# rohithr87/CILRS-Autonomous-Driving-CARLA

Measured on AMD Instinct MI355X. Metric: frames/sec CILRS train batch=128, higher is better.
Workload: dtype f32; 1 GPU; CILRS ResNet-34 train step (fwd+loss+bwd+Adam), Config A, 200x88 RGB, B=128/GPU, fp32; global_batch=128, parallelism=single

## Files before the change

### cilrs-autonomous-driving-carla_amd/cilrs_mi355/_lib.py

```python
from __future__ import annotations

import ctypes as C
import os

_HERE = os.path.dirname(os.path.abspath(__file__))
LIB_PATH = os.environ.get("CILRS_LIB") or os.path.join(_HERE, "libcilrs_hip.so")

c_float_p = C.POINTER(C.c_float)
vp = C.c_void_p
sz = C.c_size_t
i32 = C.c_int
i64 = C.c_int64
f32 = C.c_float
f64 = C.c_double
u64 = C.c_uint64


class Buffers(C.Structure):
    _fields_ = [("params", vp), ("grads", vp), ("bn_running", vp), ("bn_nbt", vp),
                ("workspace", vp)]


class AdamArgs(C.Structure):
    _fields_ = [("exp_avg", vp), ("exp_avg_sq", vp), ("lr", C.c_double), ("beta1", C.c_double),
# ... 157 lines not shown
    "cilrs_batch_assemble": (i32, [vp, i64, vp, vp, vp, vp, vp, i32, i32, i32, vp, vp, vp, vp, vp,
                                   vp]),
    "cilrs_augment_weather_u8": (i32, [vp, vp, vp, i32, i32, i32, vp, vp, vp]),
    "cilrs_batch_assemble_weather": (i32, [vp, i64, vp, vp, vp, vp, vp, vp, i32, i32, i32, vp, vp, vp,
                                           vp, vp, vp]),
    "cilrs_augment_view_u8": (i32, [vp, vp, vp, vp, i32, i32, i32, vp, vp, vp]),
    "cilrs_batch_assemble_view": (i32, [vp, i64, vp, vp, vp, vp, vp, vp, vp, i32, i32, i32, vp, vp,
                                        vp, vp, vp, vp]),
    "cilrs_replay_state_doubles": (i32, []),
    "cilrs_replay_metric_doubles": (i32, []),
    "cilrs_replay_begin": (i32, [C.POINTER(ReplayConfig), i32, i32, i64, vp, vp, vp, vp, vp, vp, vp,
                                 vp, vp]),
    "cilrs_replay_step": (i32, [C.POINTER(ReplayConfig), i32, i32, vp, vp, vp, i64, vp, vp, vp, vp,
                                vp, vp, vp, vp]),
    "cilrs_replay_finish": (i32, [C.POINTER(ReplayConfig), i32, i32, vp, vp, vp, i64, vp, vp, vp, vp,
                                  vp, vp]),
    "cilrs_eval_acc_doubles": (i32, []),
    "cilrs_eval_accumulate": (i32, [vp, vp, vp, vp, vp, i32, vp, vp, vp]),
    "cilrs_net_profile_enable": (i32, [vp, i32]),
    "cilrs_net_profile_collect": (i32, [vp]),
    "cilrs_net_profile_count": (i32, [vp]),
    "cilrs_net_profile_entry": (i32, [vp, i32, C.c_char_p, i32, C.POINTER(C.c_longlong),
                                      C.POINTER(f64), C.POINTER(f64), C.POINTER(f64)]),
    "cilrs_net_profile_reset": (i32, [vp]),
    "cilrs_conv2d_fwd": (i32, [vp, vp, vp] + [i32] * 11 + [vp, sz, vp]),
    "cilrs_conv2d_dgrad": (i32, [vp, vp, vp, vp] + [i32] * 11 + [vp, sz, vp]),
    "cilrs_conv2d_fwd_stats": (i32, [vp, vp, vp, vp, C.POINTER(i32)] + [i32] * 10 + [vp, sz, vp]),
    "cilrs_conv2d_dgrad_bnbwd": (i32, [vp] * 7 + [i32, vp, C.POINTER(i32)] + [i32] * 10
                                 + [vp, sz, vp]),
    "cilrs_conv2d_takes_classes": (i32, [i32] * 9 + [sz, i32]),
    "cilrs_conv2d_plan_info": (i32, [i32] * 9 + [sz, i32, i32] + [C.POINTER(i32)] * 4),
    "cilrs_net_conv_classes": (i32, [vp, i32, C.POINTER(i32), C.POINTER(i32)]),
    "cilrs_conv2d_wgrad_scratch_floats": (sz, [i32] * 9),
    "cilrs_conv2d_wgrad": (i32, [vp, vp, vp, vp] + [i32] * 10 + [vp]),
    "cilrs_conv2d_16_scratch_halfs": (sz, [i32] * 8),
    "cilrs_conv2d_fwd_16": (i32, [vp, vp, vp, vp] + [i32] * 9 + [vp, vp]),
    "cilrs_conv2d_dgrad_16": (i32, [vp, vp, vp, vp] + [i32] * 9 + [vp, vp]),
    "cilrs_conv2d_wgrad_16_scratch_floats": (sz, [i32] * 8),
    "cilrs_conv2d_wgrad_16": (i32, [vp, vp, vp, vp] + [i32] * 9 + [vp, vp]),
    "cilrs_conv2d_train_16": (i32, [vp] * 9 + [i32, vp] + [i32] * 12 + [vp, vp]),
    "cilrs_conv2d_infer_16": (i32, [vp] * 5 + [i32] * 11 + [vp]),
    "cilrs_stem_fold_16": (i32, [vp, vp, vp, vp, i32, vp]),
    "cilrs_stem_infer_16": (i32, [vp, vp, vp, vp, i32, i32, i32, i32, vp]),
    "cilrs_maxpool_infer_16": (i32, [vp, vp, i32, i32, i32, i32, i32, vp]),
    "cilrs_avgpool_infer_16": (i32, [vp, vp, i32, i32, i32, i32, i32, vp]),
    "cilrs_bn16_train_fwd": (i32, [vp, i32, i32, vp, vp, vp, vp, vp, C.c_float, C.c_float, vp, i32,
                                   vp, vp, vp, i32, vp]),
    "cilrs_bn16_bwd": (i32, [vp, vp, vp, i32, i32, vp, vp, i32, vp, vp, vp, vp, vp, vp, i32, vp]),
    "cilrs_conv2d_wino_split": (i32, [vp, vp, vp, vp, vp, i32, i32, i32, i32, i32, vp, sz, vp, vp, vp]),
    "cilrs_conv2d_wino_scratch_floats": (sz, [i32, i32]),
    "cilrs_conv2d_wino_fwd": (i32, [vp, vp, vp, i32, i32, i32, i32, i32, vp, vp]),
    "cilrs_conv2d_wino_fold_fwd": (i32, [vp, vp, vp, vp, vp, vp, i32, i32, i32, i32, i32, i32, i32,
                                         vp, vp]),
    "cilrs_wino_filter_transform": (i32, [vp, vp, i32, i32, i32, vp]),
    "cilrs_conv2d_wino_stamps": (i32, [vp]),
    "cilrs_conv2d_wino_pre": (i32, [vp, vp, vp, vp, i32, i32, i32, i32, i32, vp]),
    "cilrs_conv2d_wino_dgrad": (i32, [vp, vp, vp, vp, i32, i32, i32, i32, i32, vp, vp]),
    "cilrs_conv2d_wino_wgrad_scratch_floats": (sz, [i32, i32, i32, i32, i32]),
    "cilrs_conv2d_wino_wgrad": (i32, [vp, vp, vp, i32, i32, i32, i32, i32, vp, sz, vp]),
    "cilrs_bn_partial_floats": (sz, [i32]),
    "cilrs_variant_bn_stats_doubles": (sz, [i32]),
    "cilrs_variant_bn_stats_info": (i32, [i32, i32, C.POINTER(i32), C.POINTER(sz), C.POINTER(sz)]),
    "cilrs_net_bn_layer_info": (i32, [vp, i32, C.POINTER(sz), C.POINTER(i32), C.POINTER(i32),
                                      C.POINTER(i32)]),
    "cilrs_net_forward_bn_stats": (i32, [vp, C.POINTER(Buffers), vp, C.c_long, C.c_long, C.c_long, C.c_long, vp, vp]),
    "cilrs_bn_stats_finalize": (i32, [i32, vp, i32, vp, vp, vp]),
# ... 62 lines not shown
```

### cilrs-autonomous-driving-carla_amd/csrc/common.h

```cpp
#pragma once
#include <hip/hip_runtime.h>
#include <stdint.h>
#include <stddef.h>
#include "../../include/cilrs_hip.h"

namespace cilrs {

typedef float f32x4 __attribute__((ext_vector_type(4)));
typedef float f32x16 __attribute__((ext_vector_type(16)));

void set_error(const char* fmt, ...);
const char* last_error();

#define CILRS_CHECK(cond, ...)                   \
    do {                                         \
        if (!(cond)) {                           \
            ::cilrs::set_error(__VA_ARGS__);     \
            return 1;                            \
        }                                        \
    } while (0)

#define CILRS_HIP(expr)                                                                 \
    do {                                                                                \
        hipError_t e_ = (expr);                                                         \
// ... 99 lines not shown
#if defined(__HIPCC__)
__device__ __forceinline__ void wave_priority(const int mode) {
    if (mode == 0) return;
    int p;
    if (mode == 1) p = (int)(blockIdx.x >> 8) & 3;
    else p = (int)__builtin_amdgcn_s_getreg((3 << 11) | 4) & 3;
    p = __builtin_amdgcn_readfirstlane(p);
    if (p == 0) __builtin_amdgcn_s_setprio(0);
    else if (p == 1) __builtin_amdgcn_s_setprio(1);
    else if (p == 2) __builtin_amdgcn_s_setprio(2);
    else __builtin_amdgcn_s_setprio(3);
}
__device__ __forceinline__ void wave_stagger(const int mode) {
    if (mode < 16) return;
    const int units = mode - 16;
    const int k = (int)((blockIdx.x >> 8) % 5u);
    for (int i = 0; i < k * units; ++i) __builtin_amdgcn_s_sleep(1);
}
#endif
int wave_priority_mode();

struct WgradArgs {
    const float* x;
    const float* dy;
    float* dw;
    float* slabs;
    int N, H, W, Cin;
    int Ho, Wo, Cout;
    int KH, KW, stride, pad;
    int x_ld, dy_ld;
    int Cin_dst;
    int accumulate;
    int prio_mode;
};
size_t wgrad_scratch_floats(const WgradArgs& a);
int launch_conv_wgrad(const WgradArgs& a, hipStream_t s);

size_t bn_partial_floats(int C);
int launch_bn_train_fwd(const float* y, int M, int C, const float* gamma, const float* beta,
                        float* running_mean, float* running_var, long long* nbt, float momentum,
                        float eps, const float* residual, int relu, float* stats, float* partial,
                        float* z, int pre_nblk, hipStream_t s, void* z16 = nullptr,
                        double* acc_head = nullptr, double* acc = nullptr);
constexpr int kBnStatsHead = 2, kBnStatsRows = 4;
int launch_bn_train_stats(const float* y, int M, int C, double* acc, float* partial, hipStream_t s);
constexpr int kMaxConvs = 56;
struct BnEvalTable {
    int n;
    int C[kMaxConvs];
    unsigned gamma[kMaxConvs], beta[kMaxConvs];
    unsigned rm[kMaxConvs], rv[kMaxConvs];
    unsigned stats[kMaxConvs];
};
int launch_bn_eval_stats_all(const BnEvalTable& t, const float* params, const float* bn_running,
                             float* ws, float eps, hipStream_t s);
struct BnStatsTable {
    int n;
    int C[kMaxConvs];
    unsigned rm[kMaxConvs], rv[kMaxConvs];
    unsigned head[kMaxConvs], sums[kMaxConvs];
};
int launch_bn_stats_finalize(const BnStatsTable& t, const double* table, int estimator,
                             float* bn_running, long long* bn_nbt, hipStream_t s);
int launch_bn_eval_fwd(const float* y, int M, int C, const float* gamma, const float* beta,
                       const float* running_mean, const float* running_var, float eps,
                       const float* residual, int relu, float* stats, float* z, hipStream_t s);
int launch_bn_bwd(const float* dz, const float* z, const float* y, int M, int C,
                  const float* gamma, const float* stats, int relu, float* dgamma, float* dbeta,
                  int accumulate, float* coef, float* partial, float* dy, float* g_out,
// ... 567 lines not shown
```

### cilrs-autonomous-driving-carla_amd/csrc/conv_wgrad.hip

```cpp
#include "common.h"

#include <stdlib.h>

namespace cilrs {

namespace {

constexpr int BKP = 32;

template <int BT, bool TAP_UNIFORM, bool PIN>
__global__ __launch_bounds__(256, 2) void conv_wgrad_kernel(const WgradArgs a, const int Mpix,
                                                            const int splits, const int tiles_ci,
                                                            const int Ncols, const int ntiles_x,
                                                            const int ntiles_co,
                                                            const int xcd_group) {
    constexpr int WT = BT / 2, T = WT / 32;
    constexpr int QPR = BT / 4;
    constexpr int RPP = 256 / QPR;
    constexpr int PASSES = BKP / RPP;
    constexpr int PITCH = BT + 4;

    extern __shared__ __attribute__((aligned(16))) float smem[];
    float* As = smem;
    float* Bs = smem + 2 * BKP * PITCH;

    const int tid = threadIdx.x, lane = tid & 63, wave = tid >> 6;
    const int l31 = lane & 31, lh = lane >> 5;
    const int wm = wave >> 1, wn = wave & 1;
    wave_priority(a.prio_mode < 16 ? a.prio_mode : 0);

    int logical = (int)blockIdx.x;
    if (xcd_group) {
        const int nwg = (int)gridDim.x, bid = (int)blockIdx.x;
        const int q = nwg >> 3, r = nwg & 7, xcd = bid & 7;
        const int base = xcd < r ? xcd * (q + 1) : r * (q + 1) + (xcd - r) * q;
        logical = base + (bid >> 3);
    }
    const int ntile = logical % ntiles_x;
    const int co0 = ((logical / ntiles_x) % ntiles_co) * BT;
    const int z = logical / (ntiles_x * ntiles_co);

    const int KT = (Mpix + BKP - 1) / BKP;
    const int per = (KT + splits - 1) / splits;
    const int kt_begin = z * per;
    const int kt_end = min(KT, kt_begin + per);
    const int nt = max(kt_end - kt_begin, 0);

    const int q = tid % QPR, rr = tid / QPR;

    int tap, ci, col0;
    bool col_ok;
    if constexpr (TAP_UNIFORM) {
        tap = ntile / tiles_ci;
        ci = (ntile - tap * tiles_ci) * BT + q * 4;
        col0 = tap * a.Cin + (ntile - tap * tiles_ci) * BT;
        col_ok = true;
    } else {
        col0 = ntile * BT;
        const int j = col0 + q * 4;
        tap = j / a.Cin;
        ci = j - tap * a.Cin;
        col_ok = j < Ncols;
    }
    const int kh = tap / a.KW, kw = tap - kh * a.KW;
    const int HoWo = a.Ho * a.Wo;

    const int dn = BKP / HoWo, drem = BKP - dn * HoWo;
    const int doh = drem / a.Wo, dow = drem - doh * a.Wo;
    int cn[PASSES], coh[PASSES], cow[PASSES], cp[PASSES];
#pragma unroll
    for (int i = 0; i < PASSES; ++i) {
        const int p = kt_begin * BKP + rr + RPP * i;
        cp[i] = p;
        cn[i] = p / HoWo;
        const int rem = p - cn[i] * HoWo;
        coh[i] = rem / a.Wo;
        cow[i] = rem - coh[i] * a.Wo;
    }
    const __amdgpu_buffer_rsrc_t rsDy = __builtin_amdgcn_make_buffer_rsrc(
        (void*)a.dy, 0, (int)(unsigned)((size_t)Mpix * a.dy_ld * sizeof(float)), 0x00020000);
    const __amdgpu_buffer_rsrc_t rsX = __builtin_amdgcn_make_buffer_rsrc(
        (void*)a.x, 0, (int)(unsigned)((size_t)a.N * a.H * a.W * a.x_ld * sizeof(float)),
        0x00020000);
    const unsigned dyq = (unsigned)(co0 + q * 4) * 4u;
    const unsigned dy_pitch = (unsigned)a.dy_ld * 4u;

    auto load_tile = [&](f32x4(&ra)[PASSES], f32x4(&rb)[PASSES]) {
#pragma unroll
        for (int i = 0; i < PASSES; ++i) {
            const int h = coh[i] * a.stride - a.pad + kh, w = cow[i] * a.stride - a.pad + kw;
            const bool ok = col_ok && cp[i] < Mpix && h >= 0 && w >= 0 && h < a.H && w < a.W;
            const unsigned xo =
                ok ? (unsigned)(((cn[i] * a.H + h) * a.W + w) * a.x_ld + ci) * 4u : 0xFFFFFFFFu;
            ra[i] = __builtin_bit_cast(
                f32x4, __builtin_amdgcn_raw_buffer_load_b128(
                           rsDy, (int)((unsigned)cp[i] * dy_pitch + dyq), 0, 0));
            rb[i] = __builtin_bit_cast(
                f32x4, __builtin_amdgcn_raw_buffer_load_b128(rsX, (int)xo, 0, 0));
            cp[i] += BKP;
            cow[i] += dow;
            int c1 = cow[i] >= a.Wo;
            cow[i] -= c1 ? a.Wo : 0;
            coh[i] += doh + c1;
            int c2 = coh[i] >= a.Ho;
            coh[i] -= c2 ? a.Ho : 0;
            cn[i] += dn + c2;
        }
    };
    auto store_tile = [&](int buf, const f32x4(&ra)[PASSES], const f32x4(&rb)[PASSES]) {
#pragma unroll
        for (int i = 0; i < PASSES; ++i) {
            const int row = rr + RPP * i;
            *reinterpret_cast<f32x4*>(As + (buf * BKP + row) * PITCH + q * 4) = ra[i];
            *reinterpret_cast<f32x4*>(Bs + (buf * BKP + row) * PITCH + q * 4) = rb[i];
        }
    };

    f32x16 acc[T][T];
#pragma unroll
    for (int i = 0; i < T; ++i)
#pragma unroll
        for (int j = 0; j < T; ++j)
#pragma unroll
            for (int r = 0; r < 16; ++r) acc[i][j][r] = 0.f;

    auto compute = [&](int buf) {
        if constexpr (T == 2) {
            const float* Ab = As + buf * BKP * PITCH + lh * PITCH + wm * WT + 2 * l31;
            const float* Bb = Bs + buf * BKP * PITCH + lh * PITCH + wn * WT + 2 * l31;
#pragma unroll
            for (int s = 0; s < BKP / 2; ++s) {
                const float2 av = *reinterpret_cast<const float2*>(Ab + 2 * s * PITCH);
                const float2 bv = *reinterpret_cast<const float2*>(Bb + 2 * s * PITCH);
                acc[0][0] = __builtin_amdgcn_mfma_f32_32x32x2f32(av.x, bv.x, acc[0][0], 0, 0, 0);
                acc[0][1] = __builtin_amdgcn_mfma_f32_32x32x2f32(av.x, bv.y, acc[0][1], 0, 0, 0);
                acc[1][0] = __builtin_amdgcn_mfma_f32_32x32x2f32(av.y, bv.x, acc[1][0], 0, 0, 0);
                acc[1][1] = __builtin_amdgcn_mfma_f32_32x32x2f32(av.y, bv.y, acc[1][1], 0, 0, 0);
            }
// ... 129 lines not shown
        __shared__ float red1[256];
        const int opb = 256 / G;
        const int g = threadIdx.x / opb, ol = threadIdx.x - g * opb;
        const size_t idx = (size_t)blockIdx.x * opb + ol;
        float v = 0.f;
        if (idx < n_src) {
            const float* base = slabs + idx;
            float acc[4] = {0.f, 0.f, 0.f, 0.f};
            int sidx = g;
            for (; sidx + 3 * G < splits; sidx += 4 * G) {
#pragma unroll
                for (int u = 0; u < 4; ++u) acc[u] += base[(size_t)(sidx + u * G) * n_src];
            }
            for (; sidx < splits; sidx += G) acc[0] += base[(size_t)sidx * n_src];
            v = (acc[0] + acc[1]) + (acc[2] + acc[3]);
        }
        if (G > 1) {
            red1[threadIdx.x] = v;
            __syncthreads();
            if (g == 0) {
                for (int k = 1; k < G; ++k) v += red1[k * opb + ol];
            }
        }
        if (g == 0 && idx < n_src) {
            const int ci = (int)(idx % cin);
            if (ci < cin_dst) {
                const size_t o = (idx / cin) * cin_dst + ci;
                dw[o] = accumulate ? dw[o] + v : v;
            }
        }
    }
}

struct WPlan { int bt; bool uniform; int tiles_ci; int ntiles; int ncols; int splits; };

double wplan_cost(double flops, int tiles, int splits, int bt, size_t out_floats) {
    static const float r128[2] = {105.f, 120.f};
    static const float r64[4] = {60.f, 85.f, 96.f, 103.f};
    const int occ = bt == 128 ? 2 : 4;
    const float* rate = bt == 128 ? r128 : r64;
    const long blocks = (long)tiles * splits;
    const long per_cu = (blocks + 255) / 256;
    const double unit = flops / (double)blocks;
    const long full = per_cu / occ, rem = per_cu % occ;
    double t = 0.0;
    if (full) t += full * unit * 256.0 * occ / (rate[occ - 1] * 1e6);
    if (rem) t += unit * 256.0 * rem / (rate[rem - 1] * 1e6);
    t += (full + (rem ? 1 : 0)) * 3.0;
    t += 4.0 + (double)out_floats * 4.0 * (2.0 * splits + 1.0) / 3.5e6;
    return t;
}

WPlan plan(const WgradArgs& a) {
    WPlan best;
    const int taps = a.KH * a.KW;
    const int Mpix = a.N * a.Ho * a.Wo;
    const int KT = cdiv(Mpix, BKP);
    const bool uniform = (a.Cin % 64) == 0;
    const size_t out_floats = (size_t)a.Cout * taps * a.Cin;
    const double flops = 2.0 * Mpix * (double)out_floats;
    static const int env_bt = experiment_env("CILRS_WGRAD_BT", 0);
    static const int env_target = experiment_env("CILRS_WGRAD_TARGET", 0);
    double bc = 1e30;
    for (int bt = 64; bt <= 128; bt += 64) {
        if (bt == 128 && !(uniform && a.Cin % 128 == 0 && a.Cout % 128 == 0)) continue;
        if (env_bt && bt != env_bt) continue;
        WPlan p;
        p.bt = bt; p.uniform = uniform; p.ncols = taps * a.Cin;
        if (uniform) { p.tiles_ci = a.Cin / bt; p.ntiles = taps * p.tiles_ci; }
        else { p.tiles_ci = 1; p.ntiles = cdiv(p.ncols, bt); }
        const int tiles = p.ntiles * (a.Cout / bt);
        const int max_splits = KT / 4 > 0 ? KT / 4 : 1;
        for (int budget = 256; budget <= 2048; budget += 256) {
            if (env_target && budget != ((env_target + 255) / 256) * 256) continue;
            int splits = budget / tiles;
            if (splits < 1) splits = 1;
            if (splits > max_splits) splits = max_splits;
            const int per = cdiv(KT, splits);
            splits = cdiv(KT, per);
            const double c = wplan_cost(flops, tiles, splits, bt, out_floats);
            if (c < bc) { bc = c; best = p; best.splits = splits; }
        }
    }
    return best;
}

}

size_t wgrad_scratch_floats(const WgradArgs& a) {
    const WPlan p = plan(a);
    return (size_t)p.splits * a.Cout * p.ncols;
}

int launch_conv_wgrad(const WgradArgs& a_in, hipStream_t s) {
    WgradArgs a = a_in;
    a.prio_mode = wave_priority_mode();
    CILRS_CHECK(a.Cout % 64 == 0, "conv_wgrad: Cout=%d must be a multiple of 64", a.Cout);
    CILRS_CHECK(a.Cin % 4 == 0 && a.x_ld % 4 == 0 && a.dy_ld % 4 == 0,
                "conv_wgrad: Cin/x_ld/dy_ld must be multiples of 4");
    CILRS_CHECK(a.slabs != nullptr, "conv_wgrad: scratch slabs missing");
    CILRS_CHECK((size_t)a.N * a.H * a.W * a.x_ld * sizeof(float) < (1ull << 32) &&
                    (size_t)a.N * a.Ho * a.Wo * a.dy_ld * sizeof(float) < (1ull << 32),
                "conv_wgrad: tensor larger than 4 GB");
    CILRS_CHECK(((uintptr_t)a.x & 15) == 0 && ((uintptr_t)a.dy & 15) == 0 &&
                    ((uintptr_t)a.slabs & 15) == 0,
                "conv_wgrad: pointers must be 16-byte aligned");
    const WPlan p = plan(a);
    const int Mpix = a.N * a.Ho * a.Wo;
    const int ntiles_co = a.Cout / p.bt;
    static const int xcd = experiment_env("CILRS_WGRAD_XCD", 1);
    dim3 grid(p.ntiles * ntiles_co * p.splits, 1, 1);
    const size_t lds = (size_t)4 * BKP * (p.bt + 4) * sizeof(float);
    static const bool pin = experiment_env("CILRS_WGRAD_PIN", 1) != 0;
    if (p.bt == 128) {
        if (set_max_dynamic_lds(reinterpret_cast<const void*>(&conv_wgrad_kernel<128, true, true>), (int)lds) ||
            set_max_dynamic_lds(reinterpret_cast<const void*>(&conv_wgrad_kernel<128, true, false>), (int)lds))
            return 1;
        if (pin)
            conv_wgrad_kernel<128, true, true><<<grid, 256, lds, s>>>(a, Mpix, p.splits,
                                                                      p.tiles_ci, p.ncols, p.ntiles, ntiles_co, xcd);
        else
            conv_wgrad_kernel<128, true, false><<<grid, 256, lds, s>>>(a, Mpix, p.splits,
                                                                       p.tiles_ci, p.ncols, p.ntiles, ntiles_co, xcd);
    } else if (p.uniform) {
        if (pin)
            conv_wgrad_kernel<64, true, true><<<grid, 256, lds, s>>>(a, Mpix, p.splits,
                                                                     p.tiles_ci, p.ncols, p.ntiles, ntiles_co, xcd);
        else
            conv_wgrad_kernel<64, true, false><<<grid, 256, lds, s>>>(a, Mpix, p.splits,
                                                                      p.tiles_ci, p.ncols, p.ntiles, ntiles_co, xcd);
    } else {
        conv_wgrad_kernel<64, false, false><<<grid, 256, lds, s>>>(a, Mpix, p.splits, p.tiles_ci,
                                                                   p.ncols, p.ntiles, ntiles_co, xcd);
    }
    CILRS_LAUNCH_CHECK();
    const size_t n_src = (size_t)a.Cout * p.ncols;
    if (a.Cin == a.Cin_dst && n_src % 4 == 0 && ((uintptr_t)a.dw & 15) == 0) {
        const size_t nvec = n_src / 4;
        int G = 1;
        while (G < 16 && nvec * G < 131072 && 8 * G <= p.splits) G *= 2;
        const int opb = 256 / G;
        wgrad_reduce_kernel<4><<<(int)((nvec + opb - 1) / opb), 256, 0, s>>>(
            a.slabs, a.dw, p.splits, n_src, a.Cin, a.Cin_dst, a.accumulate, G);
    } else {
        int G = 1;
        while (G < 16 && n_src * G < 262144 && 8 * G <= p.splits) G *= 2;
        const int opb = 256 / G;
        wgrad_reduce_kernel<1><<<(int)((n_src + opb - 1) / opb), 256, 0, s>>>(
            a.slabs, a.dw, p.splits, n_src, a.Cin, a.Cin_dst, a.accumulate, G);
    }
    CILRS_LAUNCH_CHECK();
    return 0;
}

int launch_wgrad_reduce(const float* slabs, float* dw, int splits, size_t n, int accumulate,
                        hipStream_t s) {
    CILRS_CHECK(n % 4 == 0 && ((uintptr_t)dw & 15) == 0 && ((uintptr_t)slabs & 15) == 0,
                "wgrad_reduce: n %% 4, 16-byte aligned buffers");
    const size_t nvec = n / 4;
    int G = 1;
    while (G < 16 && nvec * G < 131072 && 8 * G <= splits) G *= 2;
    const int opb = 256 / G;
    wgrad_reduce_kernel<4><<<(int)((nvec + opb - 1) / opb), 256, 0, s>>>(slabs, dw, splits, n, 0, 0,
                                                                        accumulate, G);
    CILRS_LAUNCH_CHECK();
    return 0;
// ... 4 lines not shown
```

### cilrs-autonomous-driving-carla_amd/csrc/net.hip

```cpp
#include "common.h"
#include "../../include/cilrs_hip.h"

#include <math.h>
#include <stdarg.h>
#include <stdio.h>
#include <stdlib.h>
#include <string.h>

#include <algorithm>
#include <map>
#include <memory>
#include <mutex>
#include <set>
#include <string>
#include <vector>

namespace cilrs {

static thread_local char g_err[1024] = "";
void set_error(const char* fmt, ...) {
    va_list ap;
    va_start(ap, fmt);
    vsnprintf(g_err, sizeof(g_err), fmt, ap);
    va_end(ap);
// ... 530 lines not shown
        WinoArgs wa = wino_args(net, g, c.cout, c.cin);
        wa.x = dy; wa.U = ws + net->wino_base + net->wino_table.ud[e]; wa.y = dx; wa.addend = addend;
        wa.no_tail = (overlap_configured(net) && !experiment_env("CILRS_WINO_DGRAD_TAIL", 0)) ? 1 : 0;
        wa.slabs = ws + net->ksplit; wa.slab_floats = net->ksplit_floats;
        wa.scratch_partial = ws + net->bn_partial;
        if (bwd_nblk) *bwd_nblk = 0;
        if (bn_of && bwd_nblk) {
            wa.bwd_z = ws + bn_of->z; wa.bwd_y = ws + bn_of->y; wa.bwd_stats = ws + bn_of->stats;
            wa.bwd_relu = bn_relu; wa.bwd_partial = ws + net->bn_partial;
            *bwd_nblk = wino_rows(net->B, g.H, g.W, c.cin, wa.no_tail, c.cout, net->ksplit_floats);
        }
        RUN(net, label(), conv_flops(c, g), conv_bytes(net, c, g, 4, 4, 4, true), s,
            launch_conv_wino(wa, s));
        return 0;
    }
    DgradArgs a = dgrad_args(net->B, g.H, g.W, c.cin, c.cout, c.k, c.stride, c.pad);
    a.dy = dy; a.w = w; a.dx = dx; a.addend = addend;
    if (bn_of && bwd_nblk) {
        a.bwd_z = ws + bn_of->z; a.bwd_y = ws + bn_of->y; a.bwd_stats = ws + bn_of->stats;
        a.bwd_relu = bn_relu; a.bwd_partial = ws + net->bn_partial; a.bwd_nblk = bwd_nblk;
        *bwd_nblk = 0;
    }
    a.scratch = ws + net->ksplit; a.scratch_floats = net->ksplit_floats;
    a.force_cfg = -1;
    RUN(net, label(), conv_flops(c, g), conv_bytes(net, c, g, 4, 4, 4), s, launch_conv_dgrad(a, s));
    return 0;
}

static bool wino_wgrad_on(const ConvT& c) {
    static const int env = env_int("CILRS_WINO_WGRAD", 1);
    return env != 0 && wino_wgrad_supported(c.cin, c.cout, c.k, c.stride, c.pad);
}

int conv_wgrad(cilrs_net* net, const ConvT& c, const ConvG& g, const float* x, int x_cin,
               const float* dy, float* dw, float* ws, hipStream_t s) {
    auto label = [&] { return std::string("conv_wgrad.") + kGroupName[c.group]; };
    if (x_cin == c.cin && !net->bf16_train && wino_wgrad_on(c)) {
        WinoWgradArgs wa;
        memset(&wa, 0, sizeof(wa));
        wa.x = x; wa.dy = dy; wa.dw = dw; wa.slabs = ws + net->slabs;
        wa.N = net->B; wa.H = g.H; wa.W = g.W; wa.C = c.cin; wa.K = c.cout;
        CILRS_CHECK(wino_wgrad_scratch_floats(net->B, g.H, g.W, c.cin, c.cout) <= net->slabs_floats,
                    "Winograd wgrad scratch too small");
        RUN(net, label(), conv_flops(c, g), conv_bytes(net, c, g, 4, 4, 4), s,
            launch_conv_wino_wgrad(wa, s));
        return 0;
    }
    WgradArgs a = wgrad_args(net->B, g.H, g.W, x_cin, c.cout, c.k, c.k, c.stride, c.pad, c.cin);
    a.x = x; a.dy = dy; a.dw = dw; a.slabs = ws + net->slabs;
    CILRS_CHECK(wgrad_scratch_floats(a) <= net->slabs_floats, "wgrad scratch too small");
    RUN(net, label(), conv_flops(c, g), conv_bytes(net, c, g, 4, 4, 4), s, launch_conv_wgrad(a, s));
    return 0;
}

cilrs_half* h16(float* ws, size_t off_floats) {
    return reinterpret_cast<cilrs_half*>(ws + off_floats);
}

cilrs_half* y16_of(const cilrs_net* net, float* ws, int ci) { return h16(ws, net->cg[ci].y); }

int conv_fwd16(cilrs_net* net, const ConvT& c, const ConvG& g, const cilrs_half* x16,
               float* ws, hipStream_t s, int* bn_nblk) {
    ConvF16Args a;
    memset(&a, 0, sizeof(a));
    a.x = x16; a.w = h16(ws, net->w16_all) + c.w; a.y16 = y16_of(net, ws, g.ci);
    a.bn_partial = ws + (net->side_branch == 1 ? net->bn_partial2 : net->bn_partial);
    a.N = net->B; a.H = g.H; a.W = g.W; a.Cin = c.cin; a.Ho = g.Ho; a.Wo = g.Wo; a.Cout = c.cout;
    a.K = c.k; a.stride = c.stride; a.pad = c.pad; a.bf16 = 1;
    *bn_nblk = conv_f16_train_mtiles(a);
    RUN(net, std::string("conv_fwd.") + kGroupName[c.group], conv_flops(c, g),
// ... 2807 lines not shown
    ConvPlanInfo info;
    if (dgrad) {
        if (conv_dgrad_plan_info(make_conv_dgrad(nullptr, nullptr, nullptr, nullptr, N, H, W, Cin, Cout,
                                                 K, stride, pad, force_cfg, force_splitk, scratch,
                                                 scratch_floats),
                                 &info))
            return 1;
    } else if (conv_igemm_plan_info(make_conv_fwd(nullptr, nullptr, nullptr, N, H, W, Cin, Cout, K, K,
                                                  stride, pad, force_cfg, force_splitk, scratch,
                                                  scratch_floats),
                                    &info)) {
        return 1;
    }
    *cfg = info.cfg; *splitk = info.splitk; *class_tiles = info.class_tiles;
    *parity_fused = info.parity_fused;
    return 0;
}

int cilrs_net_conv_classes(const cilrs_net* net, int conv, int* fwd, int* dgrad) {
    CILRS_CHECK(net != nullptr, "conv_classes: net is NULL");
    CILRS_CHECK(conv >= 0 && conv < (int)net->cg.size(), "conv_classes: conv %d out of range", conv);
    const ConvT& c = net->A->convs[conv];
    const ConvG& g = net->cg[conv];
    const bool igemm = conv > 0 && net->wino_slot[conv] < 0 && !net->bf16_train;
    const bool yes_f = igemm && conv_igemm_takes_classes(net->B, g.H, g.W, c.cin, c.cout, c.k, c.stride,
                                                         c.pad, false, net->ksplit_floats);
    const bool yes_d = igemm && conv_igemm_takes_classes(net->B, g.H, g.W, c.cin, c.cout, c.k, c.stride,
                                                         c.pad, true, net->ksplit_floats);
    if (fwd) *fwd = yes_f ? 1 : 0;
    if (dgrad) *dgrad = yes_d ? 1 : 0;
    return 0;
}

size_t cilrs_conv2d_wgrad_scratch_floats(int N, int H, int W, int Cin, int Cout, int KH, int KW,
                                         int stride, int pad) {
    return wgrad_scratch_floats(wgrad_args(N, H, W, Cin, Cout, KH, KW, stride, pad, Cin));
}

int cilrs_conv2d_wgrad(const float* x, const float* dy, float* dw, float* scratch, int N, int H,
                       int W, int Cin, int Cout, int KH, int KW, int stride, int pad,
                       int Cin_dst, void* stream) {
    WgradArgs a = wgrad_args(N, H, W, Cin, Cout, KH, KW, stride, pad, Cin_dst);
    a.x = x; a.dy = dy; a.dw = dw; a.slabs = scratch;
    return launch_conv_wgrad(a, reinterpret_cast<hipStream_t>(stream));
}

static size_t up8(size_t v) { return (v + 7) / 8 * 8; }
size_t cilrs_conv2d_16_scratch_halfs(int N, int H, int W, int Cin, int Cout, int K, int stride,
                                     int pad) {
    const int Ho = (H + 2 * pad - K) / stride + 1, Wo = (W + 2 * pad - K) / stride + 1;
    return up8((size_t)N * H * W * Cin) + up8((size_t)N * Ho * Wo * Cout) +
           2 * up8((size_t)Cout * K * K * Cin);
}

int cilrs_conv2d_fwd_16(const float* x, const float* w, float* y, float* bn_partial, int N, int H,
                        int W, int Cin, int Cout, int K, int stride, int pad, int bf16,
                        void* scratch16, void* stream) {
    CILRS_CHECK(x && w && y && scratch16, "conv2d_fwd_16: NULL argument");
    hipStream_t s = reinterpret_cast<hipStream_t>(stream);
    cilrs_half* x16 = reinterpret_cast<cilrs_half*>(scratch16);
    cilrs_half* w16 = x16 + up8((size_t)N * H * W * Cin);
    if (launch_f32_to_f16(x, x16, (size_t)N * H * W * Cin, bf16, s)) return 1;
    if (launch_f32_to_f16(w, w16, (size_t)Cout * K * K * Cin, bf16, s)) return 1;
    ConvF16Args a;
    memset(&a, 0, sizeof(a));
    a.x = x16; a.w = w16; a.y32 = y; a.bn_partial = bn_partial;
// ... 319 lines not shown
```

### include/cilrs_hip.h

```cpp
#ifndef CILRS_HIP_H
#define CILRS_HIP_H

#include <stddef.h>
#include <stdint.h>

#ifdef __cplusplus
extern "C" {
#endif

typedef struct cilrs_net cilrs_net;

int cilrs_version(void);
const char* cilrs_last_error(void);

int cilrs_num_params(void);
int cilrs_num_bn(void);
size_t cilrs_param_arena_floats(void);
size_t cilrs_param_count(void);
int cilrs_param_info(int i, char* name, int name_cap, size_t* offset, size_t* numel, int* ndim,
                     int* shape4);
int cilrs_bn_info(int j, char* prefix, int prefix_cap, int* channels, size_t* rm_offset,
                  size_t* rv_offset);
size_t cilrs_bn_arena_floats(void);

// ... 412 lines not shown
int cilrs_net_profile_count(const cilrs_net* net);
int cilrs_net_profile_entry(const cilrs_net* net, int i, char* label, int label_cap,
                            long long* calls, double* total_ms, double* total_flops,
                            double* total_bytes);
int cilrs_net_profile_reset(cilrs_net* net);

int cilrs_conv2d_fwd(const float* x, const float* w, float* y, int N, int H, int W, int Cin,
                     int Cout, int KH, int KW, int stride, int pad, int force_cfg,
                     int force_splitk, float* scratch, size_t scratch_floats, void* stream);
int cilrs_conv2d_dgrad(const float* dy, const float* w, float* dx, const float* addend, int N,
                       int H, int W, int Cin, int Cout, int KH, int KW, int stride, int pad,
                       int force_cfg, int force_splitk, float* scratch, size_t scratch_floats,
                       void* stream);
int cilrs_conv2d_fwd_stats(const float* x, const float* w, float* y, float* partial, int* nblk,
                           int N, int H, int W, int Cin, int Cout, int K, int stride, int pad,
                           int force_cfg, int force_splitk, float* scratch, size_t scratch_floats,
                           void* stream);
int cilrs_conv2d_dgrad_bnbwd(const float* dy, const float* w, float* dx, const float* addend,
                             const float* bwd_z, const float* bwd_y, const float* bwd_stats,
                             int bwd_relu, float* partial, int* nblk, int N, int H, int W, int Cin,
                             int Cout, int K, int stride, int pad, int force_cfg, int force_splitk,
                             float* scratch, size_t scratch_floats, void* stream);
int cilrs_conv2d_takes_classes(int N, int H, int W, int Cin, int Cout, int K, int stride, int pad,
                               int dgrad, size_t scratch_floats, int force_splitk);
int cilrs_net_conv_classes(const cilrs_net* net, int conv, int* fwd, int* dgrad);
int cilrs_conv2d_plan_info(int N, int H, int W, int Cin, int Cout, int K, int stride, int pad,
                           int dgrad, size_t scratch_floats, int force_cfg, int force_splitk,
                           int* cfg, int* splitk, int* class_tiles, int* parity_fused);
size_t cilrs_conv2d_wgrad_scratch_floats(int N, int H, int W, int Cin, int Cout, int KH, int KW,
                                         int stride, int pad);
int cilrs_conv2d_wgrad(const float* x, const float* dy, float* dw, float* scratch, int N, int H,
                       int W, int Cin, int Cout, int KH, int KW, int stride, int pad,
                       int Cin_dst, void* stream);

size_t cilrs_conv2d_16_scratch_halfs(int N, int H, int W, int Cin, int Cout, int K, int stride,
                                     int pad);
int cilrs_conv2d_fwd_16(const float* x, const float* w, float* y, float* bn_partial, int N, int H,
                        int W, int Cin, int Cout, int K, int stride, int pad, int bf16,
                        void* scratch16, void* stream);
int cilrs_conv2d_dgrad_16(const float* dy, const float* w, float* dx, const float* addend, int N,
                          int H, int W, int Cin, int Cout, int K, int stride, int pad, int bf16,
                          void* scratch16, void* stream);
size_t cilrs_conv2d_wgrad_16_scratch_floats(int N, int H, int W, int Cin, int Cout, int K,
                                            int stride, int pad);
int cilrs_conv2d_wgrad_16(const float* x, const float* dy, float* dw, float* scratch32, int N,
                          int H, int W, int Cin, int Cout, int K, int stride, int pad, int bf16,
                          void* scratch16, void* stream);

int cilrs_bn_bwd_frozen(const float* dz, const float* z, int M, int C, const float* gamma,
                        const float* stats, int relu, float* dy, float* g_out, void* stream);
int cilrs_bn_bwd_pool_frozen(const float* dpool, const uint8_t* argmax, const float* y, int N, int H,
                             int W, int C, const float* gamma, const float* stats, float* dy,
                             void* stream);

int cilrs_saliency_map(const float* dimage, long sn, long sc, long sh, long sw, int B, int H, int W,
                       const float* chan_scale3, float* heat, uint8_t* heat_u8, float* peak,
                       void* stream);

#define CILRS_ATTR_SMOOTHGRAD 0
#define CILRS_ATTR_INTEGRATED 1
int cilrs_attr_samples(const uint8_t* frames_u8, const uint8_t* baseline_u8, int B, int H, int W,
                       int mode, int S, int s_begin, int s_count, float sigma255, uint64_t seed,
                       float* out, void* stream);
int cilrs_attr_accumulate(const float* dimage, long sn, long sc, long sh, long sw, int B, int s_count,
                          int H, int W, int first, float* acc, void* stream);
int cilrs_attr_finalize(const float* acc, const uint8_t* frames_u8, const uint8_t* baseline_u8, int B,
// ... 92 lines not shown
```

Baseline: 14210 frames/s.

## Skip padded-border pixels in wgrad by iterating per-tap valid output rectangles

Adds a rectangle mode to the weight-gradient kernel: for each filter tap, only the output pixels whose input lies inside the image are reduced, and taps are ordered by descending work. The planner picks this mode when the valid work is well below the dense work and the modeled cost is lower. This is meant to remove wasted loads and FMAs on zero-padding contributions in small feature maps, at the cost of uneven per-tap work and extra index arithmetic. New API entry points expose the plan and an optional routing override for wino layers.

```diff
diff --git a/cilrs-autonomous-driving-carla_amd/cilrs_mi355/_lib.py b/cilrs-autonomous-driving-carla_amd/cilrs_mi355/_lib.py
--- a/cilrs-autonomous-driving-carla_amd/cilrs_mi355/_lib.py
+++ b/cilrs-autonomous-driving-carla_amd/cilrs_mi355/_lib.py
@@ -213,6 +213,9 @@
     "cilrs_conv2d_plan_info": (i32, [i32] * 9 + [sz, i32, i32] + [C.POINTER(i32)] * 4),
     "cilrs_net_conv_classes": (i32, [vp, i32, C.POINTER(i32), C.POINTER(i32)]),
     "cilrs_conv2d_wgrad_scratch_floats": (sz, [i32] * 9),
+    "cilrs_conv2d_wgrad_ex": (i32, [vp, vp, vp, vp] + [i32] * 12 + [vp]),
+    "cilrs_conv2d_wgrad_plan_info": (i32, [i32] * 10 + [C.POINTER(i32)] * 3),
+    "cilrs_net_wgrad_route": (i32, [vp, i32, C.POINTER(i32), C.POINTER(i32)]),
     "cilrs_conv2d_wgrad": (i32, [vp, vp, vp, vp] + [i32] * 10 + [vp]),
     "cilrs_conv2d_16_scratch_halfs": (sz, [i32] * 8),
     "cilrs_conv2d_fwd_16": (i32, [vp, vp, vp, vp] + [i32] * 9 + [vp, vp]),
diff --git a/cilrs-autonomous-driving-carla_amd/csrc/common.h b/cilrs-autonomous-driving-carla_amd/csrc/common.h
--- a/cilrs-autonomous-driving-carla_amd/csrc/common.h
+++ b/cilrs-autonomous-driving-carla_amd/csrc/common.h
@@ -155,9 +155,12 @@
     int Cin_dst;
     int accumulate;
     int prio_mode;
+    int rect_mode;
 };
 size_t wgrad_scratch_floats(const WgradArgs& a);
 int launch_conv_wgrad(const WgradArgs& a, hipStream_t s);
+void wgrad_plan_info(const WgradArgs& a, int* tile, int* splits, int* rect);
+int wgrad_rect_env();
 
 size_t bn_partial_floats(int C);
 int launch_bn_train_fwd(const float* y, int M, int C, const float* gamma, const float* beta,
diff --git a/cilrs-autonomous-driving-carla_amd/csrc/conv_wgrad.hip b/cilrs-autonomous-driving-carla_amd/csrc/conv_wgrad.hip
--- a/cilrs-autonomous-driving-carla_amd/csrc/conv_wgrad.hip
+++ b/cilrs-autonomous-driving-carla_amd/csrc/conv_wgrad.hip
@@ -1,6 +1,7 @@
 #include "common.h"
 
 #include <stdlib.h>
+#include <string.h>
 
 namespace cilrs {
 
@@ -8,12 +9,26 @@
 
 constexpr int BKP = 32;
 
-template <int BT, bool TAP_UNIFORM, bool PIN>
+constexpr int kRectMaxTaps = 64;
+struct WgradTapOrder { unsigned char tap[kRectMaxTaps]; };
+
+__host__ __device__ inline void rect_range(int in, int out, int k, int stride, int pad, int* o0,
+                                           int* v) {
+    const int lo = pad - k, hi = in - 1 + pad - k;
+    const int b = lo > 0 ? (lo + stride - 1) / stride : 0;
+    const int e = hi < 0 ? -1 : hi / stride < out - 1 ? hi / stride : out - 1;
+    *o0 = b;
+    *v = e >= b ? e - b + 1 : 0;
+}
+
+template <int BT, bool TAP_UNIFORM, bool PIN, bool RECT = false>
 __global__ __launch_bounds__(256, 2) void conv_wgrad_kernel(const WgradArgs a, const int Mpix,
                                                             const int splits, const int tiles_ci,
                                                             const int Ncols, const int ntiles_x,
                                                             const int ntiles_co,
-                                                            const int xcd_group) {
+                                                            const int xcd_group,
+                                                            const WgradTapOrder ord) {
+    static_assert(!RECT || TAP_UNIFORM, "rectangle mode needs a block-uniform tap");
     constexpr int WT = BT / 2, T = WT / 32;
     constexpr int QPR = BT / 4;
     constexpr int RPP = 256 / QPR;
@@ -36,11 +51,29 @@
         const int base = xcd < r ? xcd * (q + 1) : r * (q + 1) + (xcd - r) * q;
         logical = base + (bid >> 3);
     }
-    const int ntile = logical % ntiles_x;
-    const int co0 = ((logical / ntiles_x) % ntiles_co) * BT;
-    const int z = logical / (ntiles_x * ntiles_co);
-
-    const int KT = (Mpix + BKP - 1) / BKP;
+    int ntile, co0, z;
+    if constexpr (RECT) {
+        const int per_tap = tiles_ci * ntiles_co * splits;
+        const int rank = logical / per_tap, r = logical - rank * per_tap;
+        ntile = (int)ord.tap[rank] * tiles_ci + r % tiles_ci;
+        co0 = ((r / tiles_ci) % ntiles_co) * BT;
+        z = r / (tiles_ci * ntiles_co);
+    } else {
+        ntile = logical % ntiles_x;
+        co0 = ((logical / ntiles_x) % ntiles_co) * BT;
+        z = logical / (ntiles_x * ntiles_co);
+    }
+
+    int oh0 = 0, ow0 = 0, rh = a.Ho, rw = a.Wo, Mc = Mpix;
+    if constexpr (RECT) {
+        const int tap_b = ntile / tiles_ci;
+        rect_range(a.H, a.Ho, tap_b / a.KW, a.stride, a.pad, &oh0, &rh);
+        rect_range(a.W, a.Wo, tap_b % a.KW, a.stride, a.pad, &ow0, &rw);
+        Mc = a.N * rh * rw;
+        if (Mc == 0) rh = rw = 1;
+    }
+
+    const int KT = (Mc + BKP - 1) / BKP;
     const int per = (KT + splits - 1) / splits;
     const int kt_begin = z * per;
     const int kt_end = min(KT, kt_begin + per);
@@ -63,10 +96,10 @@
         col_ok = j < Ncols;
     }
     const int kh = tap / a.KW, kw = tap - kh * a.KW;
-    const int HoWo = a.Ho * a.Wo;
+    const int HoWo = rh * rw;
 
     const int dn = BKP / HoWo, drem = BKP - dn * HoWo;
-    const int doh = drem / a.Wo, dow = drem - doh * a.Wo;
+    const int doh = drem / rw, dow = drem - doh * rw;
     int cn[PASSES], coh[PASSES], cow[PASSES], cp[PASSES];
 #pragma unroll
     for (int i = 0; i < PASSES; ++i) {
@@ -74,8 +107,8 @@
         cp[i] = p;
         cn[i] = p / HoWo;
         const int rem = p - cn[i] * HoWo;
-        coh[i] = rem / a.Wo;
-        cow[i] = rem - coh[i] * a.Wo;
+        coh[i] = rem / rw;
+        cow[i] = rem - coh[i] * rw;
     }
     const __amdgpu_buffer_rsrc_t rsDy = __builtin_amdgcn_make_buffer_rsrc(
         (void*)a.dy, 0, (int)(unsigned)((size_t)Mpix * a.dy_ld * sizeof(float)), 0x00020000);
@@ -88,22 +121,27 @@
     auto load_tile = [&](f32x4(&ra)[PASSES], f32x4(&rb)[PASSES]) {
 #pragma unroll
         for (int i = 0; i < PASSES; ++i) {
-            const int h = coh[i] * a.stride - a.pad + kh, w = cow[i] * a.stride - a.pad + kw;
-            const bool ok = col_ok && cp[i] < Mpix && h >= 0 && w >= 0 && h < a.H && w < a.W;
+            const int oh = oh0 + coh[i], ow = ow0 + cow[i];
+            const int h = oh * a.stride - a.pad + kh, w = ow * a.stride - a.pad + kw;
+            const bool ok = RECT ? cp[i] < Mc
+                                 : col_ok && cp[i] < Mpix && h >= 0 && w >= 0 && h < a.H && w < a.W;
             const unsigned xo =
                 ok ? (unsigned)(((cn[i] * a.H + h) * a.W + w) * a.x_ld + ci) * 4u : 0xFFFFFFFFu;
+            const unsigned dyo =
+                !RECT ? (unsigned)cp[i] * dy_pitch + dyq
+                      : ok ? (unsigned)((cn[i] * a.Ho + oh) * a.Wo + ow) * dy_pitch + dyq
+                           : 0xFFFFFFFFu;
             ra[i] = __builtin_bit_cast(
-                f32x4, __builtin_amdgcn_raw_buffer_load_b128(
-                           rsDy, (int)((unsigned)cp[i] * dy_pitch + dyq), 0, 0));
+                f32x4, __builtin_amdgcn_raw_buffer_load_b128(rsDy, (int)dyo, 0, 0));
             rb[i] = __builtin_bit_cast(
                 f32x4, __builtin_amdgcn_raw_buffer_load_b128(rsX, (int)xo, 0, 0));
             cp[i] += BKP;
             cow[i] += dow;
-            int c1 = cow[i] >= a.Wo;
-            cow[i] -= c1 ? a.Wo : 0;
+            int c1 = cow[i] >= rw;
+            cow[i] -= c1 ? rw : 0;
             coh[i] += doh + c1;
-            int c2 = coh[i] >= a.Ho;
-            coh[i] -= c2 ? a.Ho : 0;
+            int c2 = coh[i] >= rh;
+            coh[i] -= c2 ? rh : 0;
             cn[i] += dn + c2;
         }
     };
@@ -299,7 +337,38 @@
     }
 }
 
-struct WPlan { int bt; bool uniform; int tiles_ci; int ntiles; int ncols; int splits; };
+struct WPlan {
+    int bt; bool uniform; int tiles_ci; int ntiles; int ncols; int splits;
+    bool rect;
+    int dense_splits;
+    WgradTapOrder ord;
+};
+
+int rect_env() {
+    static const int env = env_int("CILRS_WGRAD_RECT", 1);
+    return env;
+}
+bool rect_env_on() { return rect_env() != 0; }
+
+struct RectTiles { long sum; int max; WgradTapOrder ord; };
+RectTiles rect_tiles(const WgradArgs& a) {
+    RectTiles r;
+    memset(&r, 0, sizeof(r));
+    const int taps = a.KH * a.KW;
+    int kt[kRectMaxTaps];
+    for (int t = 0; t < taps; ++t) {
+        int o0, vh, vw;
+        rect_range(a.H, a.Ho, t / a.KW, a.stride, a.pad, &o0, &vh);
+        rect_range(a.W, a.Wo, t % a.KW, a.stride, a.pad, &o0, &vw);
+        kt[t] = cdiv(a.N * vh * vw, BKP);
+        r.sum += kt[t];
+        if (kt[t] > r.max) r.max = kt[t];
+        int i = t;
+        for (; i > 0 && kt[r.ord.tap[i - 1]] < kt[t]; --i) r.ord.tap[i] = r.ord.tap[i - 1];
+        r.ord.tap[i] = (unsigned char)t;
+    }
+    return r;
+}
 
 double wplan_cost(double flops, int tiles, int splits, int bt, size_t out_floats) {
     static const float r128[2] = {105.f, 120.f};
@@ -320,6 +389,7 @@
 
 WPlan plan(const WgradArgs& a) {
     WPlan best;
+    memset(&best, 0, sizeof(best));
     const int taps = a.KH * a.KW;
     const int Mpix = a.N * a.Ho * a.Wo;
     const int KT = cdiv(Mpix, BKP);
@@ -329,10 +399,12 @@
     static const int env_bt = experiment_env("CILRS_WGRAD_BT", 0);
     static const int env_target = experiment_env("CILRS_WGRAD_TARGET", 0);
     double bc = 1e30;
+    double dense_cost[2] = {1e30, 1e30};
     for (int bt = 64; bt <= 128; bt += 64) {
         if (bt == 128 && !(uniform && a.Cin % 128 == 0 && a.Cout % 128 == 0)) continue;
         if (env_bt && bt != env_bt) continue;
         WPlan p;
+        memset(&p, 0, sizeof(p));
         p.bt = bt; p.uniform = uniform; p.ncols = taps * a.Cin;
         if (uniform) { p.tiles_ci = a.Cin / bt; p.ntiles = taps * p.tiles_ci; }
         else { p.tiles_ci = 1; p.ntiles = cdiv(p.ncols, bt); }
@@ -346,7 +418,37 @@
             const int per = cdiv(KT, splits);
             splits = cdiv(KT, per);
             const double c = wplan_cost(flops, tiles, splits, bt, out_floats);
+            if (c < dense_cost[bt / 128]) dense_cost[bt / 128] = c;
             if (c < bc) { bc = c; best = p; best.splits = splits; }
+        }
+    }
+    best.dense_splits = best.splits;
+    const bool can = uniform && taps <= kRectMaxTaps && a.pad > 0;
+    const bool forced = a.rect_mode >= 2;
+    if (!can || a.rect_mode == 1 || (!forced && !rect_env_on())) return best;
+    const RectTiles rt = rect_tiles(a);
+    if (!forced && rt.sum * 8 > (long)taps * KT * 7) return best;
+    const double rflops = flops * (double)rt.sum / ((double)taps * KT);
+    const WPlan dense = best;
+    double rc = forced ? 1e30 : bc;
+    for (int bt = 64; bt <= 128; bt += 64) {
+        if (bt == 128 && !(a.Cin % 128 == 0 && a.Cout % 128 == 0)) continue;
+        if (env_bt && bt != env_bt) continue;
+        WPlan p = dense;
+        p.bt = bt; p.tiles_ci = a.Cin / bt; p.ntiles = taps * p.tiles_ci;
+        p.rect = true; p.ord = rt.ord;
+        const int tiles = p.ntiles * (a.Cout / bt);
+        int max_splits = rt.max / 4 > 0 ? rt.max / 4 : 1;
+        if (max_splits > dense.splits) max_splits = dense.splits;
+        for (int budget = 256; budget <= 2048; budget += 256) {
+            int splits = budget / tiles;
+            if (splits < 1) splits = 1;
+            if (splits > max_splits) splits = max_splits;
+            const int per = cdiv(rt.max, splits);
+            splits = cdiv(rt.max, per);
+            const double c = wplan_cost(rflops, tiles, splits, bt, out_floats);
+            if (!forced && c >= dense_cost[bt / 128]) continue;
+            if (c < rc) { rc = c; best = p; best.splits = splits; }
         }
     }
     return best;
@@ -356,7 +458,16 @@
 
 size_t wgrad_scratch_floats(const WgradArgs& a) {
     const WPlan p = plan(a);
-    return (size_t)p.splits * a.Cout * p.ncols;
+    return (size_t)p.dense_splits * a.Cout * p.ncols;
+}
+
+int wgrad_rect_env() { return rect_env(); }
+
+void wgrad_plan_info(const WgradArgs& a, int* tile, int* splits, int* rect) {
+    const WPlan p = plan(a);
+    if (tile) *tile = p.bt;
+    if (splits) *splits = p.splits;
+    if (rect) *rect = p.rect ? 1 : 0;
 }
 
 int launch_conv_wgrad(const WgradArgs& a_in, hipStream_t s) {
@@ -376,29 +487,41 @@
     const int Mpix = a.N * a.Ho * a.Wo;
     const int ntiles_co = a.Cout / p.bt;
     static const int xcd = experiment_env("CILRS_WGRAD_XCD", 1);
+    static const int rect_xcd = env_int("CILRS_WGRAD_RECT_XCD", 0);
     dim3 grid(p.ntiles * ntiles_co * p.splits, 1, 1);
     const size_t lds = (size_t)4 * BKP * (p.bt + 4) * sizeof(float);
     static const bool pin = experiment_env("CILRS_WGRAD_PIN", 1) != 0;
-    if (p.bt == 128) {
+    if (p.rect) {
+        const int rx = a.rect_mode == 3 ? 1 : a.rect_mode == 2 ? 0 : rect_xcd;
+        if (p.bt == 128) {
+            if (set_max_dynamic_lds(reinterpret_cast<const void*>(&conv_wgrad_kernel<128, true, true, true>), (int)lds))
+                return 1;
+            conv_wgrad_kernel<128, true, true, true><<<grid, 256, lds, s>>>(
+                a, Mpix, p.splits, p.tiles_ci, p.ncols, p.ntiles, ntiles_co, rx, p.ord);
+        } else {
+            conv_wgrad_kernel<64, true, true, true><<<grid, 256, lds, s>>>(
+                a, Mpix, p.splits, p.tiles_ci, p.ncols, p.ntiles, ntiles_co, rx, p.ord);
+        }
+    } else if (p.bt == 128) {
         if (set_max_dynamic_lds(reinterpret_cast<const void*>(&conv_wgrad_kernel<128, true, true>), (int)lds) ||
             set_max_dynamic_lds(reinterpret_cast<const void*>(&conv_wgrad_kernel<128, true, false>), (int)lds))
             return 1;
         if (pin)
             conv_wgrad_kernel<128, true, true><<<grid, 256, lds, s>>>(a, Mpix, p.splits,
-                                                                      p.tiles_ci, p.ncols, p.ntiles, ntiles_co, xcd);
+                                                                      p.tiles_ci, p.ncols, p.ntiles, ntiles_co, xcd, p.ord);
         else
             conv_wgrad_kernel<128, true, false><<<grid, 256, lds, s>>>(a, Mpix, p.splits,
-                                                                       p.tiles_ci, p.ncols, p.ntiles, ntiles_co, xcd);
+                                                                       p.tiles_ci, p.ncols, p.ntiles, ntiles_co, xcd, p.ord);
     } else if (p.uniform) {
         if (pin)
             conv_wgrad_kernel<64, true, true><<<grid, 256, lds, s>>>(a, Mpix, p.splits,
-                                                                     p.tiles_ci, p.ncols, p.ntiles, ntiles_co, xcd);
+                                                                     p.tiles_ci, p.ncols, p.ntiles, ntiles_co, xcd, p.ord);
         else
             conv_wgrad_kernel<64, true, false><<<grid, 256, lds, s>>>(a, Mpix, p.splits,
-                                                                      p.tiles_ci, p.ncols, p.ntiles, ntiles_co, xcd);
+                                                                      p.tiles_ci, p.ncols, p.ntiles, ntiles_co, xcd, p.ord);
     } else {
         conv_wgrad_kernel<64, false, false><<<grid, 256, lds, s>>>(a, Mpix, p.splits, p.tiles_ci,
-                                                                   p.ncols, p.ntiles, ntiles_co, xcd);
+                                                                   p.ncols, p.ntiles, ntiles_co, xcd, p.ord);
     }
     CILRS_LAUNCH_CHECK();
     const size_t n_src = (size_t)a.Cout * p.ncols;
diff --git a/cilrs-autonomous-driving-carla_amd/csrc/net.hip b/cilrs-autonomous-driving-carla_amd/csrc/net.hip
--- a/cilrs-autonomous-driving-carla_amd/csrc/net.hip
+++ b/cilrs-autonomous-driving-carla_amd/csrc/net.hip
@@ -586,10 +586,25 @@
     return env != 0 && wino_wgrad_supported(c.cin, c.cout, c.k, c.stride, c.pad);
 }
 
+constexpr int kRectRouteMaxMap = 32;
+constexpr int kRectRouteMinCh = 512;
+static bool wgrad_rect_route(int B, const ConvT& c, const ConvG& g) {
+    if (wgrad_rect_env() < 2 || g.H * g.W > kRectRouteMaxMap || c.cin < kRectRouteMinCh ||
+        c.cout < kRectRouteMinCh)
+        return false;
+    int rect = 0;
+    wgrad_plan_info(wgrad_args(B, g.H, g.W, c.cin, c.cout, c.k, c.k, c.stride, c.pad, c.cin), nullptr,
+                    nullptr, &rect);
+    return rect != 0;
+}
+static int wgrad_route(const cilrs_net* net, const ConvT& c, const ConvG& g, int x_cin) {
+    return x_cin == c.cin && !net->bf16_train && wino_wgrad_on(c) && !wgrad_rect_route(net->B, c, g) ? 0 : 1;
+}
+
 int conv_wgrad(cilrs_net* net, const ConvT& c, const ConvG& g, const float* x, int x_cin,
                const float* dy, float* dw, float* ws, hipStream_t s) {
     auto label = [&] { return std::string("conv_wgrad.") + kGroupName[c.group]; };
-    if (x_cin == c.cin && !net->bf16_train && wino_wgrad_on(c)) {
+    if (wgrad_route(net, c, g, x_cin) == 0) {
         WinoWgradArgs wa;
         memset(&wa, 0, sizeof(wa));
         wa.x = x; wa.dy = dy; wa.dw = dw; wa.slabs = ws + net->slabs;
@@ -3463,6 +3478,51 @@
     return 0;
 }
 
+int cilrs_net_wgrad_route(const cilrs_net* net, int conv, int* route, int* splits) {
+    CILRS_CHECK(net != nullptr, "wgrad_route: net is NULL");
+    CILRS_CHECK(conv >= 0 && conv < (int)net->cg.size(), "wgrad_route: conv %d out of range", conv);
+    CILRS_CHECK(!net->bf16_train, "wgrad_route: the 16-bit train mode runs other kernels");
+    const ConvT& c = net->A->convs[conv];
+    const ConvG& g = net->cg[conv];
+    const int x_cin = conv == 0 ? 4 : c.cin;
+    int r = 0, sp = 0;
+    if (wgrad_route(net, c, g, x_cin) == 0) {
+        sp = (int)(wino_wgrad_scratch_floats(net->B, g.H, g.W, c.cin, c.cout) / ((size_t)9 * c.cin * c.cout));
+    } else {
+        int rect = 0;
+        wgrad_plan_info(wgrad_args(net->B, g.H, g.W, x_cin, c.cout, c.k, c.k, c.stride, c.pad, c.cin),
+                        nullptr, &sp, &rect);
+        r = rect ? 2 : 1;
+    }
+    if (route) *route = r;
+    if (splits) *splits = sp;
+    return 0;
+}
+
+int cilrs_conv2d_wgrad_plan_info(int N, int H, int W, int Cin, int Cout, int KH, int KW, int stride,
+                                 int pad, int mode, int* tile, int* splits, int* rect) {
+    CILRS_CHECK(N >= 1 && H >= 1 && W >= 1 && KH >= 1 && KW >= 1 && stride >= 1 && pad >= 0 &&
+                    H + 2 * pad >= KH && W + 2 * pad >= KW,
+                "conv2d_wgrad_plan_info: geometry");
+    CILRS_CHECK(Cin >= 4 && Cin % 4 == 0 && Cout % 64 == 0 && Cout >= 64,
+                "conv2d_wgrad_plan_info: channel counts %d -> %d", Cin, Cout);
+    CILRS_CHECK(mode >= 0 && mode <= 3, "conv2d_wgrad_plan_info: mode %d", mode);
+    WgradArgs a = wgrad_args(N, H, W, Cin, Cout, KH, KW, stride, pad, Cin);
+    a.rect_mode = mode;
+    wgrad_plan_info(a, tile, splits, rect);
+    return 0;
+}
+
+int cilrs_conv2d_wgrad_ex(const float* x, const float* dy, float* dw, float* scratch, int N, int H,
+                          int W, int Cin, int Cout, int KH, int KW, int stride, int pad,
+                          int Cin_dst, int accumulate, int mode, void* stream) {
+    CILRS_CHECK(mode >= 0 && mode <= 3, "conv2d_wgrad_ex: mode %d", mode);
+    WgradArgs a = wgrad_args(N, H, W, Cin, Cout, KH, KW, stride, pad, Cin_dst);
+    a.x = x; a.dy = dy; a.dw = dw; a.slabs = scratch;
+    a.accumulate = accumulate ? 1 : 0; a.rect_mode = mode;
+    return launch_conv_wgrad(a, reinterpret_cast<hipStream_t>(stream));
+}
+
 size_t cilrs_conv2d_wgrad_scratch_floats(int N, int H, int W, int Cin, int Cout, int KH, int KW,
                                          int stride, int pad) {
     return wgrad_scratch_floats(wgrad_args(N, H, W, Cin, Cout, KH, KW, stride, pad, Cin));
diff --git a/include/cilrs_hip.h b/include/cilrs_hip.h
--- a/include/cilrs_hip.h
+++ b/include/cilrs_hip.h
@@ -468,6 +468,12 @@
 int cilrs_conv2d_wgrad(const float* x, const float* dy, float* dw, float* scratch, int N, int H,
                        int W, int Cin, int Cout, int KH, int KW, int stride, int pad,
                        int Cin_dst, void* stream);
+int cilrs_conv2d_wgrad_ex(const float* x, const float* dy, float* dw, float* scratch, int N, int H,
+                          int W, int Cin, int Cout, int KH, int KW, int stride, int pad,
+                          int Cin_dst, int accumulate, int mode, void* stream);
+int cilrs_conv2d_wgrad_plan_info(int N, int H, int W, int Cin, int Cout, int KH, int KW, int stride,
+                                 int pad, int mode, int* tile, int* splits, int* rect);
+int cilrs_net_wgrad_route(const cilrs_net* net, int conv, int* route, int* splits);
 
 size_t cilrs_conv2d_16_scratch_halfs(int N, int H, int W, int Cin, int Cout, int K, int stride,
                                      int pad);
```

Result: no change. 14230 frames/s, median of 6 (+0.2%).
